# pixeli99/SVD_Xtend

Hardware: NVIDIA H100
Metric: SVD UNet train-step frames/sec @ 14x320x512 bf16 (higher is better)
Workload: dtype bf16

## Files before the change

svd_xtend_b200/csrc/attention.cu:

```cuda
#include "common.cuh"
#include "../../include/svd_xtend_b200.h"
#include "host_util.h"

namespace svdx {

constexpr int AT_THREADS = 288;
constexpr int AT_PRODUCER = 8;
constexpr int AT_CONSUMER_WARPS = 8;
constexpr int TILE_BYTES = 128 * 64 * 2;
constexpr float LOG2E = 1.4426950408889634f;

struct AttnKParams {
  CUtensorMap tq, tk, tv, tdo;
  int heads, S, G, RT, inner_groups, tiles, gshift, gmask;
  long long outer_stride, inner_stride, tok_stride;
  float scale;
  bf16* o; long long ldo;
  float* lse;
  float* delta;
  bf16* dq; long long lddq;
  bf16* dk; long long lddk;
  bf16* dv; long long lddv;
};

struct RowInfo {
  long long token;
  int g;
  bool valid;
};

SVDX_DEVINL RowInfo row_info(const AttnKParams& p, int r, int tile, int outer, int inner0) {
  RowInfo ri;
  const int t = tile * p.RT + (r >> p.gshift);
  ri.g = r & p.gmask;
  ri.valid = t < p.S;
  ri.token = (long long)outer * p.outer_stride + (long long)(inner0 + ri.g) * p.inner_stride + (long long)t * p.tok_stride;
  return ri;
}

SVDX_DEVINL float fast_exp2(float x) {
  float y;
  asm("ex2.approx.ftz.f32 %0, %1;" : "=f"(y) : "f"(x));
  return y;
}

SVDX_DEVINL void mma_abt64(float (&d)[32], uint32_t a_rows, uint32_t b_rows) {
  const uint64_t a = make_smem_desc_sw128(a_rows, 16, 1024), b = make_smem_desc_sw128(b_rows, 16, 1024);
  wgmma_fence();
#pragma unroll
  for (int ks = 0; ks < 4; ++ks) wgmma_ss_n64<0, 0>(d, a + 2 * ks, b + 2 * ks, ks > 0 ? 1u : 0u);
  wgmma_commit();
}
SVDX_DEVINL void mma_pb64(float (&acc)[32], const float (&p)[32], uint32_t b_rows) {
  const uint64_t b = make_smem_desc_sw128(b_rows, 8192, 1024);
  wgmma_fence();
#pragma unroll
  for (int ks = 0; ks < 4; ++ks)
    wgmma_rs_n64_tb(acc, pack_bf16x2(p[8 * ks], p[8 * ks + 1]), pack_bf16x2(p[8 * ks + 2], p[8 * ks + 3]),
                    pack_bf16x2(p[8 * ks + 4], p[8 * ks + 5]), pack_bf16x2(p[8 * ks + 6], p[8 * ks + 7]), b + (2048 >> 4) * ks, 1u);
  wgmma_commit();
}
SVDX_DEVINL int frag_col(int i, int lane) { return 8 * (i >> 2) + 2 * (lane & 3) + (i & 1); }
SVDX_DEVINL int frag_hi(int i) { return (i >> 1) & 1; }
SVDX_DEVINL float quad_max(float v) { return fmaxf(fmaxf(v, __shfl_xor_sync(0xffffffffu, v, 1)), __shfl_xor_sync(0xffffffffu, fmaxf(v, __shfl_xor_sync(0xffffffffu, v, 1)), 2)); }
SVDX_DEVINL float quad_sum(float v) { v += __shfl_xor_sync(0xffffffffu, v, 1); return v + __shfl_xor_sync(0xffffffffu, v, 2); }

SVDX_DEVINL void store_frag_rows(bf16* row_lo, bf16* row_hi, const float (&d)[32], float inv_lo, float inv_hi, int lane) {
#pragma unroll
  for (int j = 0; j < 8; ++j) {
    const int c = 8 * j + 2 * (lane & 3);
    if (row_lo) *reinterpret_cast<uint32_t*>(row_lo + c) = pack_bf16x2(d[4 * j] * inv_lo, d[4 * j + 1] * inv_lo);
    if (row_hi) *reinterpret_cast<uint32_t*>(row_hi + c) = pack_bf16x2(d[4 * j + 2] * inv_hi, d[4 * j + 3] * inv_hi);
  }
}

SVDX_DEVINL void decode_block(const AttnKParams& p, int& tile, int& head, int& outer, int& inner0) {
  tile = blockIdx.x;
  head = blockIdx.y;
  outer = blockIdx.z / p.inner_groups;
  inner0 = (blockIdx.z % p.inner_groups) * p.G;
}

SVDX_DEVINL void release(uint32_t bar, int lane) {
  __syncwarp();
  if (lane == 0) mbar_arrive(bar);
}

constexpr int FWD_KV_STAGES = 2;
constexpr int FWD_SMEM = 1024 + TILE_BYTES + FWD_KV_STAGES * 2 * TILE_BYTES + 256;

__global__ void __launch_bounds__(AT_THREADS, 1) attn_fwd_kernel(const __grid_constant__ AttnKParams p) {
  extern __shared__ uint8_t smem_raw[];
  const uint32_t base = (smem_u32(smem_raw) + 1023u) & ~1023u;
  const uint32_t sQ = base;
  const uint32_t sKV = sQ + TILE_BYTES;
  const uint32_t sBar = sKV + FWD_KV_STAGES * 2 * TILE_BYTES;
  const uint32_t b_qfull = sBar;
  const uint32_t b_kvfull = sBar + 8;
  const uint32_t b_kvempty = sBar + 8 * 3;

  const int warp = threadIdx.x >> 5, lane = threadIdx.x & 31;
  int tile, head, outer, inner0;
  decode_block(p, tile, head, outer, inner0);
  const int nkv = p.tiles;

  if (warp == AT_PRODUCER && lane == 0) {
    prefetch_tmap(&p.tq); prefetch_tmap(&p.tk); prefetch_tmap(&p.tv);
    mbar_init(b_qfull, 1);
    for (int i = 0; i < FWD_KV_STAGES; ++i) { mbar_init(b_kvfull + 8 * i, 1); mbar_init(b_kvempty + 8 * i, AT_CONSUMER_WARPS); }
    fence_barrier_init();
  }
  __syncthreads();

  if (warp == AT_PRODUCER) {
    if (lane == 0) {
      mbar_expect_tx(b_qfull, TILE_BYTES);
      tma_load_4d(&p.tq, b_qfull, sQ, head * 64, inner0, tile * p.RT, outer);
      for (int j = 0; j < nkv; ++j) {
        const int st = j % FWD_KV_STAGES;
        mbar_wait_mma(b_kvempty + 8 * st, ((j / FWD_KV_STAGES) & 1) ^ 1);
        mbar_expect_tx(b_kvfull + 8 * st, 2 * TILE_BYTES);
        tma_load_4d(&p.tk, b_kvfull + 8 * st, sKV + st * 2 * TILE_BYTES, head * 64, inner0, j * p.RT, outer);
        tma_load_4d(&p.tv, b_kvfull + 8 * st, sKV + st * 2 * TILE_BYTES + TILE_BYTES, head * 64, inner0, j * p.RT, outer);
      }
    }
    return;
  }
  const int wg = warp >> 2;
  const int r_lo = wg * 64 + (warp & 3) * 16 + (lane >> 2);
  const RowInfo ri[2] = {row_info(p, r_lo, tile, outer, inner0), row_info(p, r_lo + 8, tile, outer, inner0)};
  const float sc = p.scale * LOG2E;
  float m_run[2] = {-INFINITY, -INFINITY}, l_run[2] = {0.f, 0.f};
  float o[32];
#pragma unroll
  for (int i = 0; i < 32; ++i) o[i] = 0.f;
  mbar_wait_mma(b_qfull, 0);
  for (int j = 0; j < nkv; ++j) {
    const int st = j % FWD_KV_STAGES;
    const uint32_t sK = sKV + st * 2 * TILE_BYTES, sV = sK + TILE_BYTES;
    mbar_wait_mma(b_kvfull + 8 * st, (j / FWD_KV_STAGES) & 1);
    float s0[32], s1[32];
    mma_abt64(s0, sQ + wg * 8192, sK);
    mma_abt64(s1, sQ + wg * 8192, sK + 8192);
    wgmma_wait<0>();
    reg_fence(s0); reg_fence(s1);
    const int kvalid = p.S - j * p.RT;
    if (!(p.G == 1 && kvalid >= 128)) {
#pragma unroll
      for (int i = 0; i < 32; ++i) {
        const int c0 = frag_col(i, lane), c1 = 64 + c0;
        const RowInfo& r = ri[frag_hi(i)];
        if (!(((c0 & p.gmask) == r.g) && ((c0 >> p.gshift) < kvalid))) s0[i] = -INFINITY;
        if (!(((c1 & p.gmask) == r.g) && ((c1 >> p.gshift) < kvalid))) s1[i] = -INFINITY;
      }
    }
    float bm[2] = {-INFINITY, -INFINITY};
#pragma unroll
    for (int i = 0; i < 32; ++i) bm[frag_hi(i)] = fmaxf(bm[frag_hi(i)], fmaxf(s0[i], s1[i]));
    float msc[2], alpha[2];
#pragma unroll
    for (int h = 0; h < 2; ++h) {
      const float m_new = fmaxf(m_run[h], quad_max(bm[h]));
      const float m_use = m_new == -INFINITY ? 0.f : m_new;
      alpha[h] = fast_exp2((m_run[h] - m_use) * sc);
      m_run[h] = m_new;
      msc[h] = m_use * sc;
      l_run[h] *= alpha[h];
    }
#pragma unroll
    for (int i = 0; i < 32; ++i) {
      const int h = frag_hi(i);
      o[i] *= alpha[h];
      s0[i] = fast_exp2(fmaf(s0[i], sc, -msc[h]));
      s1[i] = fast_exp2(fmaf(s1[i], sc, -msc[h]));
      l_run[h] += s0[i] + s1[i];
    }
    mma_pb64(o, s0, sV);
    mma_pb64(o, s1, sV + 8192);
    wgmma_wait<0>();
    reg_fence(o);
    release(b_kvempty + 8 * st, lane);
  }
  bf16* rows[2];
  float inv[2];
#pragma unroll
  for (int h = 0; h < 2; ++h) {
    const float l = quad_sum(l_run[h]);
    const float m_use = m_run[h] == -INFINITY ? 0.f : m_run[h];
    inv[h] = 1.f / l;
    rows[h] = ri[h].valid ? p.o + ri[h].token * p.ldo + head * 64 : nullptr;
    if (ri[h].valid && p.lse && (lane & 3) == 0) p.lse[ri[h].token * p.heads + head] = m_use * p.scale + __logf(l);
  }
  store_frag_rows(rows[0], rows[1], o, inv[0], inv[1], lane);
}

constexpr int BWD_STAGES = 2;
constexpr int BDQ_SMEM = 1024 + 2 * TILE_BYTES + BWD_STAGES * 2 * TILE_BYTES + 256;

__global__ void __launch_bounds__(AT_THREADS, 1) attn_bwd_dq_kernel(const __grid_constant__ AttnKParams p) {
  extern __shared__ uint8_t smem_raw[];
  const uint32_t base = (smem_u32(smem_raw) + 1023u) & ~1023u;
  const uint32_t sQ = base, sDO = sQ + TILE_BYTES;
  const uint32_t sKV = sDO + TILE_BYTES;
  const uint32_t sBar = sKV + BWD_STAGES * 2 * TILE_BYTES;
  const uint32_t b_qfull = sBar;
  const uint32_t b_kvfull = sBar + 8;
  const uint32_t b_kvempty = sBar + 8 * 3;

  const int warp = threadIdx.x >> 5, lane = threadIdx.x & 31;
  int tile, head, outer, inner0;
  decode_block(p, tile, head, outer, inner0);
  const int nkv = p.tiles;

  if (warp == AT_PRODUCER && lane == 0) {
    prefetch_tmap(&p.tq); prefetch_tmap(&p.tk); prefetch_tmap(&p.tv); prefetch_tmap(&p.tdo);
    mbar_init(b_qfull, 1);
    for (int i = 0; i < BWD_STAGES; ++i) { mbar_init(b_kvfull + 8 * i, 1); mbar_init(b_kvempty + 8 * i, AT_CONSUMER_WARPS); }
    fence_barrier_init();
  }
  __syncthreads();

  if (warp == AT_PRODUCER) {
    if (lane == 0) {
      mbar_expect_tx(b_qfull, 2 * TILE_BYTES);
      tma_load_4d(&p.tq, b_qfull, sQ, head * 64, inner0, tile * p.RT, outer);
      tma_load_4d(&p.tdo, b_qfull, sDO, head * 64, inner0, tile * p.RT, outer);
      for (int j = 0; j < nkv; ++j) {
        const int st = j % BWD_STAGES;
        mbar_wait_mma(b_kvempty + 8 * st, ((j / BWD_STAGES) & 1) ^ 1);
        mbar_expect_tx(b_kvfull + 8 * st, 2 * TILE_BYTES);
        tma_load_4d(&p.tk, b_kvfull + 8 * st, sKV + st * 2 * TILE_BYTES, head * 64, inner0, j * p.RT, outer);
        tma_load_4d(&p.tv, b_kvfull + 8 * st, sKV + st * 2 * TILE_BYTES + TILE_BYTES, head * 64, inner0, j * p.RT, outer);
      }
    }
    return;
  }
  const int wg = warp >> 2;
  const int r_lo = wg * 64 + (warp & 3) * 16 + (lane >> 2);
  const RowInfo ri[2] = {row_info(p, r_lo, tile, outer, inner0), row_info(p, r_lo + 8, tile, outer, inner0)};
  const float sc = p.scale * LOG2E;
  float lse2[2], dlt[2];
#pragma unroll
  for (int h = 0; h < 2; ++h) {
    lse2[h] = ri[h].valid ? p.lse[ri[h].token * p.heads + head] * LOG2E : 0.f;
    dlt[h] = ri[h].valid ? p.delta[ri[h].token * p.heads + head] : 0.f;
  }
  float dq[32];
#pragma unroll
  for (int i = 0; i < 32; ++i) dq[i] = 0.f;
  mbar_wait_mma(b_qfull, 0);
  for (int j = 0; j < nkv; ++j) {
    const int st = j % BWD_STAGES;
    const uint32_t sK = sKV + st * 2 * TILE_BYTES, sV = sK + TILE_BYTES;
    mbar_wait_mma(b_kvfull + 8 * st, (j / BWD_STAGES) & 1);
    const int kvalid = p.S - j * p.RT;
    const bool nomask = (p.G == 1) && (kvalid >= 128);
#pragma unroll 1
    for (int kh = 0; kh < 2; ++kh) {
      float s[32], dp[32];
      mma_abt64(s, sQ + wg * 8192, sK + kh * 8192);
      mma_abt64(dp, sDO + wg * 8192, sV + kh * 8192);
      wgmma_wait<0>();
      reg_fence(s); reg_fence(dp);
#pragma unroll
      for (int i = 0; i < 32; ++i) {
        const int c = kh * 64 + frag_col(i, lane), h = frag_hi(i);
        const bool ok = ri[h].valid && (nomask || (((c & p.gmask) == ri[h].g) && ((c >> p.gshift) < kvalid)));
        const float pr = ok ? fast_exp2(fmaf(s[i], sc, -lse2[h])) * p.scale : 0.f;
        s[i] = pr * (dp[i] - dlt[h]);
      }
      mma_pb64(dq, s, sK + kh * 8192);
      wgmma_wait<0>();
      reg_fence(dq);
    }
    release(b_kvempty + 8 * st, lane);
  }
  store_frag_rows(ri[0].valid ? p.dq + ri[0].token * p.lddq + head * 64 : nullptr,
                  ri[1].valid ? p.dq + ri[1].token * p.lddq + head * 64 : nullptr, dq, 1.f, 1.f, lane);
}

constexpr int BKV_SMEM = 1024 + 2 * TILE_BYTES + BWD_STAGES * 2 * TILE_BYTES + 1024 + 256;

__global__ void __launch_bounds__(AT_THREADS, 1) attn_bwd_dkv_kernel(const __grid_constant__ AttnKParams p) {
  extern __shared__ uint8_t smem_raw[];
  const uint32_t base = (smem_u32(smem_raw) + 1023u) & ~1023u;
  const uint32_t sK = base, sV = sK + TILE_BYTES;
  const uint32_t sQD = sV + TILE_BYTES;
  const uint32_t sVec = sQD + BWD_STAGES * 2 * TILE_BYTES;
  const uint32_t sBar = sVec + 1024;
  const uint32_t b_kvfull = sBar;
  const uint32_t b_qfull = sBar + 8;
  const uint32_t b_qempty = sBar + 8 * 3;
  float* vec = reinterpret_cast<float*>(smem_raw + (sVec - smem_u32(smem_raw)));

  const int warp = threadIdx.x >> 5, lane = threadIdx.x & 31;
  int tile, head, outer, inner0;
  decode_block(p, tile, head, outer, inner0);
  const int nq = p.tiles;

  if (warp == AT_PRODUCER && lane == 0) {
    prefetch_tmap(&p.tq); prefetch_tmap(&p.tk); prefetch_tmap(&p.tv); prefetch_tmap(&p.tdo);
    mbar_init(b_kvfull, 1);
    for (int i = 0; i < BWD_STAGES; ++i) { mbar_init(b_qfull + 8 * i, 1); mbar_init(b_qempty + 8 * i, AT_CONSUMER_WARPS); }
    fence_barrier_init();
  }
  __syncthreads();

  if (warp == AT_PRODUCER) {
    if (lane == 0) {
      mbar_expect_tx(b_kvfull, 2 * TILE_BYTES);
      tma_load_4d(&p.tk, b_kvfull, sK, head * 64, inner0, tile * p.RT, outer);
      tma_load_4d(&p.tv, b_kvfull, sV, head * 64, inner0, tile * p.RT, outer);
      for (int i = 0; i < nq; ++i) {
        const int st = i % BWD_STAGES;
        mbar_wait_mma(b_qempty + 8 * st, ((i / BWD_STAGES) & 1) ^ 1);
        mbar_expect_tx(b_qfull + 8 * st, 2 * TILE_BYTES);
        tma_load_4d(&p.tq, b_qfull + 8 * st, sQD + st * 2 * TILE_BYTES, head * 64, inner0, i * p.RT, outer);
        tma_load_4d(&p.tdo, b_qfull + 8 * st, sQD + st * 2 * TILE_BYTES + TILE_BYTES, head * 64, inner0, i * p.RT, outer);
      }
    }
    return;
  }
  const int wg = warp >> 2;
  const int r_lo = wg * 64 + (warp & 3) * 16 + (lane >> 2);
  const RowInfo ki[2] = {row_info(p, r_lo, tile, outer, inner0), row_info(p, r_lo + 8, tile, outer, inner0)};
  const float sc = p.scale * LOG2E;
  const int vr = threadIdx.x & 127;
  auto load_stat = [&](int i) -> float {
    const RowInfo qi = row_info(p, vr, i, outer, inner0);
    if (threadIdx.x < 128) return qi.valid ? p.lse[qi.token * p.heads + head] * LOG2E : INFINITY;
    return qi.valid ? p.delta[qi.token * p.heads + head] : 0.f;
  };
  float stat = load_stat(0);
  float dv[32], dk[32];
#pragma unroll
  for (int i = 0; i < 32; ++i) { dv[i] = 0.f; dk[i] = 0.f; }
  mbar_wait_mma(b_kvfull, 0);
  for (int i = 0; i < nq; ++i) {
    named_bar_sync(1, 32 * AT_CONSUMER_WARPS);
    vec[threadIdx.x] = stat;
    named_bar_sync(1, 32 * AT_CONSUMER_WARPS);
    if (i + 1 < nq) stat = load_stat(i + 1);
    const int st = i % BWD_STAGES;
    const uint32_t sQ = sQD + st * 2 * TILE_BYTES, sDO = sQ + TILE_BYTES;
    mbar_wait_mma(b_qfull + 8 * st, (i / BWD_STAGES) & 1);
#pragma unroll 1
    for (int qh = 0; qh < 2; ++qh) {
      float s[32], dp[32];
      mma_abt64(s, sK + wg * 8192, sQ + qh * 8192);
      mma_abt64(dp, sV + wg * 8192, sDO + qh * 8192);
      wgmma_wait<0>();
      reg_fence(s); reg_fence(dp);
#pragma unroll
      for (int k = 0; k < 32; ++k) {
        const int c = qh * 64 + frag_col(k, lane);
        const RowInfo& r = ki[frag_hi(k)];
        const bool ok = r.valid && (p.G == 1 || (c & p.gmask) == r.g);
        const float pr = ok ? fast_exp2(fmaf(s[k], sc, -vec[c])) : 0.f;
        s[k] = pr;
        dp[k] = (pr * p.scale) * (dp[k] - vec[128 + c]);
      }
      mma_pb64(dv, s, sDO + qh * 8192);
      mma_pb64(dk, dp, sQ + qh * 8192);
      wgmma_wait<0>();
      reg_fence(dv); reg_fence(dk);
    }
    release(b_qempty + 8 * st, lane);
  }
  store_frag_rows(ki[0].valid ? p.dv + ki[0].token * p.lddv + head * 64 : nullptr,
                  ki[1].valid ? p.dv + ki[1].token * p.lddv + head * 64 : nullptr, dv, 1.f, 1.f, lane);
  store_frag_rows(ki[0].valid ? p.dk + ki[0].token * p.lddk + head * 64 : nullptr,
                  ki[1].valid ? p.dk + ki[1].token * p.lddk + head * 64 : nullptr, dk, 1.f, 1.f, lane);
}

__global__ void attn_delta_kernel(const bf16* __restrict__ o, long long ldo, const bf16* __restrict__ dout, long long lddo, long long tokens,
                                  int heads, float* __restrict__ delta) {
  const long long w = ((long long)blockIdx.x * blockDim.x + threadIdx.x) >> 5;
  const int lane = threadIdx.x & 31;
  if (w >= tokens * heads) return;
  const long long tok = w / heads;
  const int h = (int)(w - tok * heads);
  const float2 a = unpack_bf16x2(*reinterpret_cast<const uint32_t*>(o + tok * ldo + h * 64 + 2 * lane));
  const float2 b = unpack_bf16x2(*reinterpret_cast<const uint32_t*>(dout + tok * lddo + h * 64 + 2 * lane));
  const float s = warp_sum(a.x * b.x + a.y * b.y);
  if (lane == 0) delta[w] = s;
}

}

using namespace svdx;

static int attn_make_map(CUtensorMap* m, const void* ptr, int64_t ld, int cols, const SvdxAttn* d, int G, int RT) {
  const int outer = d->nseq / d->inner;
  uint64_t dims[4] = {(uint64_t)cols, (uint64_t)d->inner, (uint64_t)d->S, (uint64_t)outer};
  uint64_t strides[3] = {(uint64_t)(d->inner_stride * ld * 2), (uint64_t)(d->tok_stride * ld * 2), (uint64_t)(d->outer_stride * ld * 2)};
  if (d->inner == 1) strides[0] = (uint64_t)ld * 2;
  uint32_t box[4] = {64, (uint32_t)G, (uint32_t)RT, 1};
  return svdx_make_tmap(m, ptr, 4, dims, strides, box);
}

static int attn_setup(const SvdxAttn* d, AttnKParams& p, bool bwd, dim3& grid) {
  if (!d || !d->q || !d->k || !d->v) return svdx_fail(SVDX_E_BADARG, "attention: null pointer");
  if (d->heads <= 0 || d->S <= 0 || d->nseq <= 0 || d->inner <= 0 || d->nseq % d->inner) return svdx_fail(SVDX_E_BADARG, "attention: bad sequence geometry");
  if ((d->ldq % 8) || (d->ldk % 8) || (d->ldv % 8)) return svdx_fail(SVDX_E_BADARG, "attention: leading dims must be multiples of 8");
  memset(&p, 0, sizeof(p));
  int G = 1;
  if (d->inner > 1) {
    G = 1;
    while (G * 2 * d->S <= 128 && d->inner % (G * 2) == 0 && G < 64) G *= 2;
  }
  const int RT = 128 / G;
  if (d->inner > 1 && d->S > RT) return svdx_fail(SVDX_E_BADARG, "attention: strided sequences longer than 128 tokens are not supported");
  p.G = G; p.RT = RT; p.S = d->S; p.heads = d->heads;
  p.gmask = G - 1; p.gshift = 0;
  while ((1 << p.gshift) < G) ++p.gshift;
  p.inner_groups = d->inner / G;
  p.tiles = (d->S + RT - 1) / RT;
  p.outer_stride = d->outer_stride; p.inner_stride = d->inner_stride; p.tok_stride = d->tok_stride;
  p.scale = d->scale;
  const int cols = d->heads * 64;
  int rc;
  if ((rc = attn_make_map(&p.tq, d->q, d->ldq, cols, d, G, RT))) return rc;
  if ((rc = attn_make_map(&p.tk, d->k, d->ldk, cols, d, G, RT))) return rc;
  if ((rc = attn_make_map(&p.tv, d->v, d->ldv, cols, d, G, RT))) return rc;
  if (bwd) {
    if (!d->dout || !d->dq || !d->dk || !d->dv || !d->lse || !d->delta || !d->o) return svdx_fail(SVDX_E_BADARG, "attention_bwd: null pointer");
    if ((d->lddo % 8) || (d->lddq % 8) || (d->lddk % 8) || (d->lddv % 8) || (d->ldo % 8)) return svdx_fail(SVDX_E_BADARG, "attention_bwd: leading dims");
    if ((rc = attn_make_map(&p.tdo, d->dout, d->lddo, cols, d, G, RT))) return rc;
  } else {
    if (!d->o || (d->ldo % 8)) return svdx_fail(SVDX_E_BADARG, "attention_fwd: output");
  }
  p.o = reinterpret_cast<bf16*>(d->o); p.ldo = d->ldo;
  p.lse = d->lse; p.delta = d->delta;
  p.dq = reinterpret_cast<bf16*>(d->dq); p.lddq = d->lddq;
  p.dk = reinterpret_cast<bf16*>(d->dk); p.lddk = d->lddk;
  p.dv = reinterpret_cast<bf16*>(d->dv); p.lddv = d->lddv;
  const long long gz = (long long)(d->nseq / d->inner) * p.inner_groups;
  if (gz > 65535 || d->heads > 65535) return svdx_fail(SVDX_E_BADARG, "attention: grid too large");
  grid = dim3(p.tiles, d->heads, (unsigned)gz);
  return 0;
}

bool svdx_attention_small_eligible(const SvdxAttn* d);
int svdx_attention_small_fwd(const SvdxAttn* d, cudaStream_t st);
int svdx_attention_small_bwd(const SvdxAttn* d, cudaStream_t st);

extern "C" int svdx_attention_fwd(const SvdxAttn* d, void* stream_v) {
  cudaStream_t st = reinterpret_cast<cudaStream_t>(stream_v);
  if (svdx_attention_small_eligible(d)) return svdx_attention_small_fwd(d, st);
  AttnKParams p;
  dim3 grid;
  int rc = attn_setup(d, p, false, grid);
  if (rc) return rc;
  static bool attr[SVDX_MAX_DEVICES] = {false};
  const int slot = svdx_device_slot();
  if (!attr[slot]) {
    cudaError_t e = cudaFuncSetAttribute(attn_fwd_kernel, cudaFuncAttributeMaxDynamicSharedMemorySize, FWD_SMEM);
    if (e != cudaSuccess) return svdx_fail_cuda(e, "attention_fwd: smem attribute");
    attr[slot] = true;
  }
  attn_fwd_kernel<<<grid, AT_THREADS, FWD_SMEM, st>>>(p);
  SVDX_CHECK_LAUNCH("attention_fwd");
  return SVDX_OK;
}

extern "C" int svdx_attention_bwd(const SvdxAttn* d, void* stream_v) {
  cudaStream_t st = reinterpret_cast<cudaStream_t>(stream_v);
  if (svdx_attention_small_eligible(d)) return svdx_attention_small_bwd(d, st);
  AttnKParams p;
  dim3 grid;
  int rc = attn_setup(d, p, true, grid);
  if (rc) return rc;
  static bool attr[SVDX_MAX_DEVICES] = {false};
  const int slot = svdx_device_slot();
  if (!attr[slot]) {
    cudaError_t e = cudaFuncSetAttribute(attn_bwd_dq_kernel, cudaFuncAttributeMaxDynamicSharedMemorySize, BDQ_SMEM);
    if (e == cudaSuccess) e = cudaFuncSetAttribute(attn_bwd_dkv_kernel, cudaFuncAttributeMaxDynamicSharedMemorySize, BKV_SMEM);
    if (e != cudaSuccess) return svdx_fail_cuda(e, "attention_bwd: smem attribute");
    attr[slot] = true;
  }
  const long long tokens = (long long)d->nseq * d->S;
  const long long warps = tokens * d->heads;
  attn_delta_kernel<<<(unsigned)((warps * 32 + 255) / 256), 256, 0, st>>>(reinterpret_cast<const bf16*>(d->o), d->ldo,
                                                                         reinterpret_cast<const bf16*>(d->dout), d->lddo, tokens, d->heads, d->delta);
  attn_bwd_dq_kernel<<<grid, AT_THREADS, BDQ_SMEM, st>>>(p);
  attn_bwd_dkv_kernel<<<grid, AT_THREADS, BKV_SMEM, st>>>(p);
  SVDX_CHECK_LAUNCH("attention_bwd");
  return SVDX_OK;
}
```

svd_xtend_b200/csrc/common.cuh:

```cuda
#pragma once
#include <cuda.h>
#include <cuda_bf16.h>
#include <cuda_runtime.h>
#include <stdint.h>
#include <stdio.h>

#include "wgmma.cuh"

namespace svdx {

typedef __nv_bfloat16 bf16;

#define SVDX_DEVINL __device__ __forceinline__

#ifndef SVDX_WAIT_TIMEOUT_CYCLES
#define SVDX_WAIT_TIMEOUT_CYCLES (4000000000ll)
#endif

SVDX_DEVINL uint32_t smem_u32(const void* p) { return (uint32_t)__cvta_generic_to_shared(p); }

SVDX_DEVINL uint32_t lane_id() { return threadIdx.x & 31; }

SVDX_DEVINL bool elect_one() {
  uint32_t pred = 0;
  asm volatile(
      "{\n\t.reg .pred P;\n\t"
      "elect.sync _|P, 0xffffffff;\n\t"
      "selp.u32 %0, 1, 0, P;\n\t}\n"
      : "=r"(pred));
  return pred != 0;
}

SVDX_DEVINL void mbar_init(uint32_t bar, uint32_t count) {
  asm volatile("mbarrier.init.shared::cta.b64 [%0], %1;" ::"r"(bar), "r"(count) : "memory");
}
SVDX_DEVINL void fence_barrier_init() {
  asm volatile("fence.mbarrier_init.release.cluster;" ::: "memory");
}
SVDX_DEVINL void fence_proxy_async_smem() {
  asm volatile("fence.proxy.async.shared::cta;" ::: "memory");
}
SVDX_DEVINL void mbar_expect_tx(uint32_t bar, uint32_t bytes) {
  asm volatile("mbarrier.arrive.expect_tx.shared::cta.b64 _, [%0], %1;" ::"r"(bar), "r"(bytes) : "memory");
}
SVDX_DEVINL void mbar_arrive(uint32_t bar) {
  asm volatile("mbarrier.arrive.shared::cta.b64 _, [%0];" ::"r"(bar) : "memory");
}
SVDX_DEVINL bool mbar_try_wait(uint32_t bar, uint32_t parity) {
  uint32_t ok;
  asm volatile(
      "{\n\t.reg .pred P;\n\t"
      "mbarrier.try_wait.parity.shared::cta.b64 P, [%1], %2;\n\t"
      "selp.u32 %0, 1, 0, P;\n\t}\n"
      : "=r"(ok)
      : "r"(bar), "r"(parity)
      : "memory");
  return ok != 0;
}
SVDX_DEVINL void mbar_wait(uint32_t bar, uint32_t parity) {
  if (mbar_try_wait(bar, parity)) return;
  long long t0 = clock64();
  while (!mbar_try_wait(bar, parity)) {
    if (clock64() - t0 > SVDX_WAIT_TIMEOUT_CYCLES) {
      printf("svdx: mbarrier wait timeout block %d thread %d bar %u parity %u\n", blockIdx.x, threadIdx.x, bar, parity);
      __trap();
    }
  }
}

SVDX_DEVINL void mbar_wait_mma(uint32_t bar, uint32_t parity) {
  if (mbar_try_wait(bar, parity)) return;
  long long t0 = clock64();
  while (!mbar_try_wait(bar, parity))
    if (clock64() - t0 > SVDX_WAIT_TIMEOUT_CYCLES) __trap();
}

SVDX_DEVINL void prefetch_tmap(const CUtensorMap* m) {
  asm volatile("prefetch.tensormap [%0];" ::"l"(reinterpret_cast<uint64_t>(m)) : "memory");
}
SVDX_DEVINL void tma_load_2d(const CUtensorMap* m, uint32_t bar, uint32_t dst, int c0, int c1) {
  asm volatile(
      "cp.async.bulk.tensor.2d.shared::cluster.global.mbarrier::complete_tx::bytes [%0], [%1, {%3, %4}], [%2];"
      ::"r"(dst), "l"(reinterpret_cast<uint64_t>(m)), "r"(bar), "r"(c0), "r"(c1)
      : "memory");
}
SVDX_DEVINL void tma_load_3d(const CUtensorMap* m, uint32_t bar, uint32_t dst, int c0, int c1, int c2) {
  asm volatile(
      "cp.async.bulk.tensor.3d.shared::cluster.global.mbarrier::complete_tx::bytes [%0], [%1, {%3, %4, %5}], [%2];"
      ::"r"(dst), "l"(reinterpret_cast<uint64_t>(m)), "r"(bar), "r"(c0), "r"(c1), "r"(c2)
      : "memory");
}
SVDX_DEVINL void tma_load_4d(const CUtensorMap* m, uint32_t bar, uint32_t dst, int c0, int c1, int c2, int c3) {
  asm volatile(
      "cp.async.bulk.tensor.4d.shared::cluster.global.mbarrier::complete_tx::bytes [%0], [%1, {%3, %4, %5, %6}], [%2];"
      ::"r"(dst), "l"(reinterpret_cast<uint64_t>(m)), "r"(bar), "r"(c0), "r"(c1), "r"(c2), "r"(c3)
      : "memory");
}
SVDX_DEVINL void tma_load_4d_im2col(const CUtensorMap* m, uint32_t bar, uint32_t dst, int c0, int c1, int c2, int c3, uint16_t ow,
                                    uint16_t oh) {
  asm volatile(
      "cp.async.bulk.tensor.4d.shared::cluster.global.im2col.mbarrier::complete_tx::bytes [%0], [%1, {%3, %4, %5, %6}], [%2], {%7, %8};"
      ::"r"(dst), "l"(reinterpret_cast<uint64_t>(m)), "r"(bar), "r"(c0), "r"(c1), "r"(c2), "r"(c3), "h"(ow), "h"(oh)
      : "memory");
}

SVDX_DEVINL void tma_store_3d(const CUtensorMap* m, uint32_t src, int c0, int c1, int c2) {
  asm volatile("cp.async.bulk.tensor.3d.global.shared::cta.bulk_group [%0, {%2, %3, %4}], [%1];"
               ::"l"(reinterpret_cast<uint64_t>(m)), "r"(src), "r"(c0), "r"(c1), "r"(c2)
               : "memory");
}
SVDX_DEVINL void tma_store_4d(const CUtensorMap* m, uint32_t src, int c0, int c1, int c2, int c3) {
  asm volatile("cp.async.bulk.tensor.4d.global.shared::cta.bulk_group [%0, {%2, %3, %4, %5}], [%1];"
               ::"l"(reinterpret_cast<uint64_t>(m)), "r"(src), "r"(c0), "r"(c1), "r"(c2), "r"(c3)
               : "memory");
}
SVDX_DEVINL void tma_reduce_add_3d(const CUtensorMap* m, uint32_t src, int c0, int c1, int c2) {
  asm volatile("cp.reduce.async.bulk.tensor.3d.global.shared::cta.add.bulk_group [%0, {%2, %3, %4}], [%1];"
               ::"l"(reinterpret_cast<uint64_t>(m)), "r"(src), "r"(c0), "r"(c1), "r"(c2)
               : "memory");
}
SVDX_DEVINL void bulk_commit() { asm volatile("cp.async.bulk.commit_group;" ::: "memory"); }
template <int N>
SVDX_DEVINL void bulk_wait_read() { asm volatile("cp.async.bulk.wait_group.read %0;" ::"n"(N) : "memory"); }
template <int N>
SVDX_DEVINL void bulk_wait() { asm volatile("cp.async.bulk.wait_group %0;" ::"n"(N) : "memory"); }
SVDX_DEVINL void st_shared_v4(uint32_t addr, uint32_t a, uint32_t b, uint32_t c, uint32_t d) {
  asm volatile("st.shared.v4.b32 [%0], {%1, %2, %3, %4};" ::"r"(addr), "r"(a), "r"(b), "r"(c), "r"(d) : "memory");
}

SVDX_DEVINL void wgmma_fence() { asm volatile("wgmma.fence.sync.aligned;" ::: "memory"); }
SVDX_DEVINL void wgmma_commit() { asm volatile("wgmma.commit_group.sync.aligned;" ::: "memory"); }
template <int N>
SVDX_DEVINL void wgmma_wait() { asm volatile("wgmma.wait_group.sync.aligned %0;" ::"n"(N) : "memory"); }
template <int R>
SVDX_DEVINL void reg_fence(float (&d)[R]) {
#pragma unroll
  for (int i = 0; i < R; ++i) asm volatile("" : "+f"(d[i])::"memory");
}

SVDX_DEVINL void named_bar_sync(int id, int nthreads) { asm volatile("bar.sync %0, %1;" ::"r"(id), "r"(nthreads) : "memory"); }

SVDX_DEVINL uint64_t make_smem_desc_sw128(uint32_t saddr, uint32_t lbo_bytes, uint32_t sbo_bytes) {
  uint64_t d = 0;
  d |= (uint64_t)((saddr & 0x3FFFF) >> 4);
  d |= (uint64_t)((lbo_bytes >> 4) & 0x3FFF) << 16;
  d |= (uint64_t)((sbo_bytes >> 4) & 0x3FFF) << 32;
  d |= (uint64_t)1 << 62;
  return d;
}

SVDX_DEVINL float silu_f(float x) { return __fdividef(x, 1.0f + __expf(-x)); }
SVDX_DEVINL float silu_grad_f(float x) {
  const float s = __fdividef(1.0f, 1.0f + __expf(-x));
  return s * fmaf(x, 1.0f - s, 1.0f);
}
#define SVDX_HDINL __host__ __device__ __forceinline__
SVDX_HDINL float gelu_tail_log2(float ax) {
  float p = -1.92123457e-06f;
  p = fmaf(p, ax, 6.32884985e-05f);
  p = fmaf(p, ax, -0.000943420862f);
  p = fmaf(p, ax, 0.0085562719f);
  p = fmaf(p, ax, -0.0540522821f);
  p = fmaf(p, ax, -0.458381772f);
  p = fmaf(p, ax, -1.15127838f);
  p = fmaf(p, ax, -0.999993861f);
  return p;
}
SVDX_HDINL float exp2_fast(float x) {
#ifdef __CUDA_ARCH__
  float y;
  asm("ex2.approx.ftz.f32 %0, %1;" : "=f"(y) : "f"(x));
  return y;
#else
  return exp2f(x);
#endif
}
SVDX_HDINL float normal_cdf_f(float x) {
  const float q = exp2_fast(gelu_tail_log2(fminf(fabsf(x), 5.5f)));
  return x < 0.f ? q : 1.0f - q;
}
SVDX_HDINL float gelu_erf_f(float x) { return x * normal_cdf_f(x); }
SVDX_HDINL float gelu_erf_grad_f(float x) {
  const float pdf = 0.3989422804014327f * exp2_fast(-0.72134752044448170f * x * x);
  return fmaf(x, pdf, normal_cdf_f(x));
}

SVDX_DEVINL uint32_t pack_bf16x2(float lo, float hi) {
  __nv_bfloat162 v = __floats2bfloat162_rn(lo, hi);
  return *reinterpret_cast<uint32_t*>(&v);
}
SVDX_DEVINL float2 unpack_bf16x2(uint32_t u) {
  __nv_bfloat162 v = *reinterpret_cast<__nv_bfloat162*>(&u);
  return __bfloat1622float2(v);
}

SVDX_DEVINL float warp_sum(float v) {
#pragma unroll
  for (int o = 16; o > 0; o >>= 1) v += __shfl_xor_sync(0xffffffffu, v, o);
  return v;
}
SVDX_DEVINL float warp_max(float v) {
#pragma unroll
  for (int o = 16; o > 0; o >>= 1) v = fmaxf(v, __shfl_xor_sync(0xffffffffu, v, o));
  return v;
}

}
```

Before: 159.6.

## Pipeline attention forward softmax with next QK MMA and add TMA output stores

Forward attention is restructured into a full producer warpgroup with setmaxnreg register rebalancing, deeper KV staging, and N=128 QK wgmma. The loop is software-pipelined so the P·V MMA for tile j-1 overlaps the softmax of tile j, and the output is written through swizzled shared memory with a TMA store. Backward kernels release KV buffers earlier, defer dq MMA waits, and split the dkv stats vector per warpgroup to avoid cross-warpgroup barriers. This adds register pressure and synchronisation complexity.

```diff
diff --git a/svd_xtend_b200/csrc/attention.cu b/svd_xtend_b200/csrc/attention.cu
--- a/svd_xtend_b200/csrc/attention.cu
+++ b/svd_xtend_b200/csrc/attention.cu
@@ -12,6 +12,7 @@
 
 struct AttnKParams {
   CUtensorMap tq, tk, tv, tdo;
+  CUtensorMap to;
   int heads, S, G, RT, inner_groups, tiles, gshift, gmask;
   long long outer_stride, inner_stride, tok_stride;
   float scale;
@@ -51,13 +52,21 @@
   for (int ks = 0; ks < 4; ++ks) wgmma_ss_n64<0, 0>(d, a + 2 * ks, b + 2 * ks, ks > 0 ? 1u : 0u);
   wgmma_commit();
 }
-SVDX_DEVINL void mma_pb64(float (&acc)[32], const float (&p)[32], uint32_t b_rows) {
+template <int R>
+SVDX_DEVINL void reg_fence_u(uint32_t (&d)[R]) {
+#pragma unroll
+  for (int i = 0; i < R; ++i) asm volatile("" : "+r"(d[i])::"memory");
+}
+SVDX_DEVINL void pack_frag(uint32_t (&a)[16], const float (&d)[32]) {
+#pragma unroll
+  for (int i = 0; i < 16; ++i) a[i] = pack_bf16x2(d[2 * i], d[2 * i + 1]);
+  reg_fence_u(a);
+}
+SVDX_DEVINL void mma_ab64(float (&acc)[32], const uint32_t (&a)[16], uint32_t b_rows) {
   const uint64_t b = make_smem_desc_sw128(b_rows, 8192, 1024);
   wgmma_fence();
 #pragma unroll
-  for (int ks = 0; ks < 4; ++ks)
-    wgmma_rs_n64_tb(acc, pack_bf16x2(p[8 * ks], p[8 * ks + 1]), pack_bf16x2(p[8 * ks + 2], p[8 * ks + 3]),
-                    pack_bf16x2(p[8 * ks + 4], p[8 * ks + 5]), pack_bf16x2(p[8 * ks + 6], p[8 * ks + 7]), b + (2048 >> 4) * ks, 1u);
+  for (int ks = 0; ks < 4; ++ks) wgmma_rs_n64_tb(acc, a[4 * ks], a[4 * ks + 1], a[4 * ks + 2], a[4 * ks + 3], b + (2048 >> 4) * ks, 1u);
   wgmma_commit();
 }
 SVDX_DEVINL int frag_col(int i, int lane) { return 8 * (i >> 2) + 2 * (lane & 3) + (i & 1); }
@@ -86,10 +95,27 @@
   if (lane == 0) mbar_arrive(bar);
 }
 
-constexpr int FWD_KV_STAGES = 2;
+constexpr int FWD_THREADS = 384;
+constexpr int FWD_PRODUCER_REGS = 40, FWD_CONSUMER_REGS = 232;
+constexpr int FWD_KV_STAGES = 4;
 constexpr int FWD_SMEM = 1024 + TILE_BYTES + FWD_KV_STAGES * 2 * TILE_BYTES + 256;
 
-__global__ void __launch_bounds__(AT_THREADS, 1) attn_fwd_kernel(const __grid_constant__ AttnKParams p) {
+SVDX_DEVINL void mma_abt128(float (&d)[64], uint32_t a_rows, uint32_t b_rows) {
+  const uint64_t a = make_smem_desc_sw128(a_rows, 16, 1024), b = make_smem_desc_sw128(b_rows, 16, 1024);
+  wgmma_fence();
+#pragma unroll
+  for (int ks = 0; ks < 4; ++ks) wgmma_ss_n128<0, 0>(d, a + 2 * ks, b + 2 * ks, ks > 0 ? 1u : 0u);
+  wgmma_commit();
+}
+SVDX_DEVINL void mma_pb128(float (&acc)[32], const uint32_t (&p)[32], uint32_t b_rows) {
+  const uint64_t b = make_smem_desc_sw128(b_rows, 8192, 1024);
+  wgmma_fence();
+#pragma unroll
+  for (int ks = 0; ks < 8; ++ks) wgmma_rs_n64_tb(acc, p[4 * ks], p[4 * ks + 1], p[4 * ks + 2], p[4 * ks + 3], b + (2048 >> 4) * ks, 1u);
+  wgmma_commit();
+}
+
+__global__ void __launch_bounds__(FWD_THREADS, 1) attn_fwd_kernel(const __grid_constant__ AttnKParams p) {
   extern __shared__ uint8_t smem_raw[];
   const uint32_t base = (smem_u32(smem_raw) + 1023u) & ~1023u;
   const uint32_t sQ = base;
@@ -97,23 +123,24 @@
   const uint32_t sBar = sKV + FWD_KV_STAGES * 2 * TILE_BYTES;
   const uint32_t b_qfull = sBar;
   const uint32_t b_kvfull = sBar + 8;
-  const uint32_t b_kvempty = sBar + 8 * 3;
+  const uint32_t b_kvempty = sBar + 8 * (1 + FWD_KV_STAGES);
 
   const int warp = threadIdx.x >> 5, lane = threadIdx.x & 31;
   int tile, head, outer, inner0;
   decode_block(p, tile, head, outer, inner0);
   const int nkv = p.tiles;
 
-  if (warp == AT_PRODUCER && lane == 0) {
-    prefetch_tmap(&p.tq); prefetch_tmap(&p.tk); prefetch_tmap(&p.tv);
+  if (threadIdx.x == 0) {
+    prefetch_tmap(&p.tq); prefetch_tmap(&p.tk); prefetch_tmap(&p.tv); prefetch_tmap(&p.to);
     mbar_init(b_qfull, 1);
     for (int i = 0; i < FWD_KV_STAGES; ++i) { mbar_init(b_kvfull + 8 * i, 1); mbar_init(b_kvempty + 8 * i, AT_CONSUMER_WARPS); }
     fence_barrier_init();
   }
   __syncthreads();
 
-  if (warp == AT_PRODUCER) {
-    if (lane == 0) {
+  if (warp < 4) {
+    setmaxnreg_dec<FWD_PRODUCER_REGS>();
+    if (threadIdx.x == 0) {
       mbar_expect_tx(b_qfull, TILE_BYTES);
       tma_load_4d(&p.tq, b_qfull, sQ, head * 64, inner0, tile * p.RT, outer);
       for (int j = 0; j < nkv; ++j) {
@@ -126,38 +153,32 @@
     }
     return;
   }
-  const int wg = warp >> 2;
+  setmaxnreg_inc<FWD_CONSUMER_REGS>();
+  const int wg = (warp >> 2) - 1;
   const int r_lo = wg * 64 + (warp & 3) * 16 + (lane >> 2);
   const RowInfo ri[2] = {row_info(p, r_lo, tile, outer, inner0), row_info(p, r_lo + 8, tile, outer, inner0)};
+  const uint32_t sQw = sQ + wg * 8192;
   const float sc = p.scale * LOG2E;
   float m_run[2] = {-INFINITY, -INFINITY}, l_run[2] = {0.f, 0.f};
-  float o[32];
+  float o[32], s[64], alpha[2];
+  uint32_t pb[32];
 #pragma unroll
   for (int i = 0; i < 32; ++i) o[i] = 0.f;
-  mbar_wait_mma(b_qfull, 0);
-  for (int j = 0; j < nkv; ++j) {
-    const int st = j % FWD_KV_STAGES;
-    const uint32_t sK = sKV + st * 2 * TILE_BYTES, sV = sK + TILE_BYTES;
-    mbar_wait_mma(b_kvfull + 8 * st, (j / FWD_KV_STAGES) & 1);
-    float s0[32], s1[32];
-    mma_abt64(s0, sQ + wg * 8192, sK);
-    mma_abt64(s1, sQ + wg * 8192, sK + 8192);
-    wgmma_wait<0>();
-    reg_fence(s0); reg_fence(s1);
+
+  auto softmax = [&](int j) {
     const int kvalid = p.S - j * p.RT;
     if (!(p.G == 1 && kvalid >= 128)) {
 #pragma unroll
-      for (int i = 0; i < 32; ++i) {
-        const int c0 = frag_col(i, lane), c1 = 64 + c0;
+      for (int i = 0; i < 64; ++i) {
+        const int c = frag_col(i, lane);
         const RowInfo& r = ri[frag_hi(i)];
-        if (!(((c0 & p.gmask) == r.g) && ((c0 >> p.gshift) < kvalid))) s0[i] = -INFINITY;
-        if (!(((c1 & p.gmask) == r.g) && ((c1 >> p.gshift) < kvalid))) s1[i] = -INFINITY;
+        if (!(((c & p.gmask) == r.g) && ((c >> p.gshift) < kvalid))) s[i] = -INFINITY;
       }
     }
     float bm[2] = {-INFINITY, -INFINITY};
 #pragma unroll
-    for (int i = 0; i < 32; ++i) bm[frag_hi(i)] = fmaxf(bm[frag_hi(i)], fmaxf(s0[i], s1[i]));
-    float msc[2], alpha[2];
+    for (int i = 0; i < 32; ++i) bm[frag_hi(i)] = fmaxf(bm[frag_hi(i)], fmaxf(s[i], s[i + 32]));
+    float msc[2];
 #pragma unroll
     for (int h = 0; h < 2; ++h) {
       const float m_new = fmaxf(m_run[h], quad_max(bm[h]));
@@ -170,28 +191,74 @@
 #pragma unroll
     for (int i = 0; i < 32; ++i) {
       const int h = frag_hi(i);
-      o[i] *= alpha[h];
-      s0[i] = fast_exp2(fmaf(s0[i], sc, -msc[h]));
-      s1[i] = fast_exp2(fmaf(s1[i], sc, -msc[h]));
-      l_run[h] += s0[i] + s1[i];
-    }
-    mma_pb64(o, s0, sV);
-    mma_pb64(o, s1, sV + 8192);
+      s[i] = fast_exp2(fmaf(s[i], sc, -msc[h]));
+      s[i + 32] = fast_exp2(fmaf(s[i + 32], sc, -msc[h]));
+      l_run[h] += s[i] + s[i + 32];
+    }
+  };
+  auto pack_p = [&]() {
+#pragma unroll
+    for (int i = 0; i < 32; ++i) pb[i] = pack_bf16x2(s[2 * i], s[2 * i + 1]);
+    reg_fence_u(pb);
+  };
+
+  mbar_wait_mma(b_qfull, 0);
+  mbar_wait_mma(b_kvfull, 0);
+  mma_abt128(s, sQw, sKV);
+  wgmma_wait<0>();
+  reg_fence(s);
+  softmax(0);
+  pack_p();
+  for (int j = 1; j < nkv; ++j) {
+    const int st = j % FWD_KV_STAGES, sp = (j - 1) % FWD_KV_STAGES;
+    mbar_wait_mma(b_kvfull + 8 * st, (j / FWD_KV_STAGES) & 1);
+    mma_abt128(s, sQw, sKV + st * 2 * TILE_BYTES);
+    mma_pb128(o, pb, sKV + sp * 2 * TILE_BYTES + TILE_BYTES);
+    wgmma_wait<1>();
+    reg_fence(s);
+    softmax(j);
     wgmma_wait<0>();
     reg_fence(o);
-    release(b_kvempty + 8 * st, lane);
-  }
-  bf16* rows[2];
+    reg_fence_u(pb);
+    release(b_kvempty + 8 * sp, lane);
+#pragma unroll
+    for (int i = 0; i < 32; ++i) o[i] *= alpha[frag_hi(i)];
+    reg_fence(o);
+    pack_p();
+  }
+  {
+    const int sp = (nkv - 1) % FWD_KV_STAGES;
+    mma_pb128(o, pb, sKV + sp * 2 * TILE_BYTES + TILE_BYTES);
+    wgmma_wait<0>();
+    reg_fence(o);
+    reg_fence_u(pb);
+    release(b_kvempty + 8 * sp, lane);
+  }
   float inv[2];
 #pragma unroll
   for (int h = 0; h < 2; ++h) {
     const float l = quad_sum(l_run[h]);
     const float m_use = m_run[h] == -INFINITY ? 0.f : m_run[h];
     inv[h] = 1.f / l;
-    rows[h] = ri[h].valid ? p.o + ri[h].token * p.ldo + head * 64 : nullptr;
     if (ri[h].valid && p.lse && (lane & 3) == 0) p.lse[ri[h].token * p.heads + head] = m_use * p.scale + __logf(l);
   }
-  store_frag_rows(rows[0], rows[1], o, inv[0], inv[1], lane);
+  const int rl = (warp & 3) * 16 + (lane >> 2);
+#pragma unroll
+  for (int jc = 0; jc < 8; ++jc) {
+#pragma unroll
+    for (int h = 0; h < 2; ++h) {
+      const int r = rl + 8 * h;
+      st_shared_u32(sQw + r * 128 + ((jc ^ (r & 7)) << 4) + 4 * (lane & 3),
+                    pack_bf16x2(o[4 * jc + 2 * h] * inv[h], o[4 * jc + 2 * h + 1] * inv[h]));
+    }
+  }
+  fence_proxy_async_smem();
+  named_bar_sync(1 + wg, 128);
+  if ((threadIdx.x & 127) == 0) {
+    tma_store_4d(&p.to, sQw, head * 64, inner0, tile * p.RT + wg * (p.RT >> 1), outer);
+    bulk_commit();
+    bulk_wait_read<0>();
+  }
 }
 
 constexpr int BWD_STAGES = 2;
@@ -246,6 +313,7 @@
     dlt[h] = ri[h].valid ? p.delta[ri[h].token * p.heads + head] : 0.f;
   }
   float dq[32];
+  uint32_t ds[16];
 #pragma unroll
   for (int i = 0; i < 32; ++i) dq[i] = 0.f;
   mbar_wait_mma(b_qfull, 0);
@@ -261,7 +329,8 @@
       mma_abt64(s, sQ + wg * 8192, sK + kh * 8192);
       mma_abt64(dp, sDO + wg * 8192, sV + kh * 8192);
       wgmma_wait<0>();
-      reg_fence(s); reg_fence(dp);
+      reg_fence(s); reg_fence(dp); reg_fence(dq); reg_fence_u(ds);
+      if (kh == 0 && j > 0) release(b_kvempty + 8 * ((j - 1) % BWD_STAGES), lane);
 #pragma unroll
       for (int i = 0; i < 32; ++i) {
         const int c = kh * 64 + frag_col(i, lane), h = frag_hi(i);
@@ -269,17 +338,17 @@
         const float pr = ok ? fast_exp2(fmaf(s[i], sc, -lse2[h])) * p.scale : 0.f;
         s[i] = pr * (dp[i] - dlt[h]);
       }
-      mma_pb64(dq, s, sK + kh * 8192);
-      wgmma_wait<0>();
-      reg_fence(dq);
-    }
-    release(b_kvempty + 8 * st, lane);
-  }
+      pack_frag(ds, s);
+      mma_ab64(dq, ds, sK + kh * 8192);
+    }
+  }
+  wgmma_wait<0>();
+  reg_fence(dq); reg_fence_u(ds);
   store_frag_rows(ri[0].valid ? p.dq + ri[0].token * p.lddq + head * 64 : nullptr,
                   ri[1].valid ? p.dq + ri[1].token * p.lddq + head * 64 : nullptr, dq, 1.f, 1.f, lane);
 }
 
-constexpr int BKV_SMEM = 1024 + 2 * TILE_BYTES + BWD_STAGES * 2 * TILE_BYTES + 1024 + 256;
+constexpr int BKV_SMEM = 1024 + 2 * TILE_BYTES + BWD_STAGES * 2 * TILE_BYTES + 2048 + 256;
 
 __global__ void __launch_bounds__(AT_THREADS, 1) attn_bwd_dkv_kernel(const __grid_constant__ AttnKParams p) {
   extern __shared__ uint8_t smem_raw[];
@@ -287,7 +356,7 @@
   const uint32_t sK = base, sV = sK + TILE_BYTES;
   const uint32_t sQD = sV + TILE_BYTES;
   const uint32_t sVec = sQD + BWD_STAGES * 2 * TILE_BYTES;
-  const uint32_t sBar = sVec + 1024;
+  const uint32_t sBar = sVec + 2048;
   const uint32_t b_kvfull = sBar;
   const uint32_t b_qfull = sBar + 8;
   const uint32_t b_qempty = sBar + 8 * 3;
@@ -325,22 +394,25 @@
   const int r_lo = wg * 64 + (warp & 3) * 16 + (lane >> 2);
   const RowInfo ki[2] = {row_info(p, r_lo, tile, outer, inner0), row_info(p, r_lo + 8, tile, outer, inner0)};
   const float sc = p.scale * LOG2E;
-  const int vr = threadIdx.x & 127;
-  auto load_stat = [&](int i) -> float {
-    const RowInfo qi = row_info(p, vr, i, outer, inner0);
-    if (threadIdx.x < 128) return qi.valid ? p.lse[qi.token * p.heads + head] * LOG2E : INFINITY;
-    return qi.valid ? p.delta[qi.token * p.heads + head] : 0.f;
+  const int t = threadIdx.x & 127;
+  float* wvec = vec + 256 * wg;
+  auto load_stat = [&](int i, float& l2, float& dl) {
+    const RowInfo qi = row_info(p, t, i, outer, inner0);
+    l2 = qi.valid ? p.lse[qi.token * p.heads + head] * LOG2E : INFINITY;
+    dl = qi.valid ? p.delta[qi.token * p.heads + head] : 0.f;
   };
-  float stat = load_stat(0);
+  float st_l, st_d;
+  load_stat(0, st_l, st_d);
   float dv[32], dk[32];
 #pragma unroll
   for (int i = 0; i < 32; ++i) { dv[i] = 0.f; dk[i] = 0.f; }
   mbar_wait_mma(b_kvfull, 0);
   for (int i = 0; i < nq; ++i) {
-    named_bar_sync(1, 32 * AT_CONSUMER_WARPS);
-    vec[threadIdx.x] = stat;
-    named_bar_sync(1, 32 * AT_CONSUMER_WARPS);
-    if (i + 1 < nq) stat = load_stat(i + 1);
+    named_bar_sync(1 + wg, 128);
+    wvec[t] = st_l;
+    wvec[128 + t] = st_d;
+    named_bar_sync(1 + wg, 128);
+    if (i + 1 < nq) load_stat(i + 1, st_l, st_d);
     const int st = i % BWD_STAGES;
     const uint32_t sQ = sQD + st * 2 * TILE_BYTES, sDO = sQ + TILE_BYTES;
     mbar_wait_mma(b_qfull + 8 * st, (i / BWD_STAGES) & 1);
@@ -356,14 +428,17 @@
         const int c = qh * 64 + frag_col(k, lane);
         const RowInfo& r = ki[frag_hi(k)];
         const bool ok = r.valid && (p.G == 1 || (c & p.gmask) == r.g);
-        const float pr = ok ? fast_exp2(fmaf(s[k], sc, -vec[c])) : 0.f;
+        const float pr = ok ? fast_exp2(fmaf(s[k], sc, -wvec[c])) : 0.f;
         s[k] = pr;
-        dp[k] = (pr * p.scale) * (dp[k] - vec[128 + c]);
+        dp[k] = (pr * p.scale) * (dp[k] - wvec[128 + c]);
       }
-      mma_pb64(dv, s, sDO + qh * 8192);
-      mma_pb64(dk, dp, sQ + qh * 8192);
+      uint32_t pt[16], dst[16];
+      pack_frag(pt, s);
+      pack_frag(dst, dp);
+      mma_ab64(dv, pt, sDO + qh * 8192);
+      mma_ab64(dk, dst, sQ + qh * 8192);
       wgmma_wait<0>();
-      reg_fence(dv); reg_fence(dk);
+      reg_fence(dv); reg_fence(dk); reg_fence_u(pt); reg_fence_u(dst);
     }
     release(b_qempty + 8 * st, lane);
   }
@@ -429,6 +504,7 @@
     if ((rc = attn_make_map(&p.tdo, d->dout, d->lddo, cols, d, G, RT))) return rc;
   } else {
     if (!d->o || (d->ldo % 8)) return svdx_fail(SVDX_E_BADARG, "attention_fwd: output");
+    if ((rc = attn_make_map(&p.to, d->o, d->ldo, cols, d, G, RT / 2))) return rc;
   }
   p.o = reinterpret_cast<bf16*>(d->o); p.ldo = d->ldo;
   p.lse = d->lse; p.delta = d->delta;
@@ -459,7 +535,7 @@
     if (e != cudaSuccess) return svdx_fail_cuda(e, "attention_fwd: smem attribute");
     attr[slot] = true;
   }
-  attn_fwd_kernel<<<grid, AT_THREADS, FWD_SMEM, st>>>(p);
+  attn_fwd_kernel<<<grid, FWD_THREADS, FWD_SMEM, st>>>(p);
   SVDX_CHECK_LAUNCH("attention_fwd");
   return SVDX_OK;
 }
diff --git a/svd_xtend_b200/csrc/common.cuh b/svd_xtend_b200/csrc/common.cuh
--- a/svd_xtend_b200/csrc/common.cuh
+++ b/svd_xtend_b200/csrc/common.cuh
@@ -124,6 +124,7 @@
 SVDX_DEVINL void bulk_wait_read() { asm volatile("cp.async.bulk.wait_group.read %0;" ::"n"(N) : "memory"); }
 template <int N>
 SVDX_DEVINL void bulk_wait() { asm volatile("cp.async.bulk.wait_group %0;" ::"n"(N) : "memory"); }
+SVDX_DEVINL void st_shared_u32(uint32_t addr, uint32_t a) { asm volatile("st.shared.b32 [%0], %1;" ::"r"(addr), "r"(a) : "memory"); }
 SVDX_DEVINL void st_shared_v4(uint32_t addr, uint32_t a, uint32_t b, uint32_t c, uint32_t d) {
   asm volatile("st.shared.v4.b32 [%0], {%1, %2, %3, %4};" ::"r"(addr), "r"(a), "r"(b), "r"(c), "r"(d) : "memory");
 }
@@ -139,6 +140,11 @@
 }
 
 SVDX_DEVINL void named_bar_sync(int id, int nthreads) { asm volatile("bar.sync %0, %1;" ::"r"(id), "r"(nthreads) : "memory"); }
+
+template <int R>
+SVDX_DEVINL void setmaxnreg_dec() { asm volatile("setmaxnreg.dec.sync.aligned.u32 %0;" ::"n"(R)); }
+template <int R>
+SVDX_DEVINL void setmaxnreg_inc() { asm volatile("setmaxnreg.inc.sync.aligned.u32 %0;" ::"n"(R)); }
 
 SVDX_DEVINL uint64_t make_smem_desc_sw128(uint32_t saddr, uint32_t lbo_bytes, uint32_t sbo_bytes) {
   uint64_t d = 0;
```

Result: no change. 160.0 (median of 6 runs) (+0.3%).
